# Amano-Ginji/distributed-tensorflow-example

Measured on AMD Instinct MI355X. Metric: samples/sec (whole node) MNIST MLP sync-SGD at 1/2/4/8 MI355X; step-time p50, higher is better.
Workload: dtype fp32; 1 GPU; model=mlp-784-100-10 (example.py), global_batch=100, per_gpu_batch=100, parallelism=dp1, optimizer=sgd lr=0.0005, grad_allreduce=none, engine=persistent-fp32, exchange_mode=persistent, launch=single process, steps_per_launch=550, hipgraph_steps=0, input_prefetch=in-kernel copier workgroups, activation=sigmoid

## Files before the change

### csrc/kernels/mlp_persist_f32.hip

```cpp
#include "common.h"
#include "mlp_api.h"

#include <atomic>

#include <cstdlib>

namespace dtfk {
namespace mlpf {

typedef __attribute__((ext_vector_type(4))) uint32_t u32x4;
typedef __attribute__((address_space(1))) unsigned gu32;

constexpr int DIN = 784, HID = 100, NCLS = 10;
constexpr int NJ = 7;
constexpr int NQ = 4;
constexpr int NTW = 2;
constexpr int NBT = 7;
constexpr int BROWS = 16 * NBT;
constexpr int XTS = 128;
constexpr int NCOMP = NJ * NQ;
constexpr int THREADS = 512;
constexpr int NCOP = 16;
constexpr int NCOPR = 14;
constexpr int RES_LR_BYTE = 124;
// ... 324 lines not shown
}

__device__ void copier(const Args& a, int cid, uint8_t* smem) {
  const int tid = threadIdx.x;
  const int B = a.B;
  if (tid == 0) { PRO(NCOMP + cid, 0); }
  for (int st = cid; st < a.next_steps; st += NCOP) {
    const uint8_t* src = a.host_next + (long long)st * a.rec_h;
    uint8_t* dst = a.stage_next + (long long)st * REC;
    constexpr int C16 = DIN / 16;
    for (int k = tid; k < BROWS * C16; k += THREADS) {
      const int row = k / C16, c = k % C16;
      uint4 v = make_uint4(0u, 0u, 0u, 0u);
      if (row < B) v = reinterpret_cast<const uint4*>(src)[row * C16 + c];
      *reinterpret_cast<uint4*>(smem + row * CROW + 16 * c) = v;
    }
    if (tid < 128) dst[XROW_BYTES + tid] = tid < B ? src[(long long)B * DIN + tid] : (uint8_t)0;
    __syncthreads();
    for (int k = tid; k < BROWS * C16; k += THREADS) {
      const int row = k / C16, c = k % C16;
      reinterpret_cast<uint4*>(dst)[row * C16 + c] = *reinterpret_cast<const uint4*>(smem + row * CROW + 16 * c);
    }
    __syncthreads();
  }
  if (tid == 0) { PRO(NCOMP + cid, 1); }
}

__device__ void copier_res(const Args& a, int cid, uint8_t* smem) {
  if (cid >= NCOPR) return;
  const int tid = threadIdx.x;
  constexpr int RR = 8;
  int* dec = reinterpret_cast<int*>(smem + RR * CROW);
  const int B = a.B;
  const int hb = (int)(2 * a.rec_h);
  const auto hrs = __builtin_amdgcn_make_buffer_rsrc(const_cast<uint8_t*>(a.host_recs), 0, hb, 0x00020000);
  for (int st = 0;; ++st) {
    const long long k = a.run0 + st;
    if (tid == 0) {
      int d = 1;
      const long long t0 = (long long)__builtin_amdgcn_s_memrealtime();
      const long long lim = cid == 0 ? a.idle : a.idle + a.timeout;
      for (;;) {
        const long long v = __hip_atomic_load(a.door, __ATOMIC_RELAXED, __HIP_MEMORY_SCOPE_SYSTEM);
        if (v < 0) { d = 0; break; }
        if (v > k) break;
        if (cid != 0 && __hip_atomic_load(a.dctr + 16, __ATOMIC_RELAXED, __HIP_MEMORY_SCOPE_AGENT) != 0u) { d = 0; break; }
        if ((long long)__builtin_amdgcn_s_memrealtime() - t0 > lim) { d = 0; break; }
        __builtin_amdgcn_s_sleep(1);
      }
      if (cid == 0 && !d) __hip_atomic_store(a.dctr + 16, 1u, __ATOMIC_RELAXED, __HIP_MEMORY_SCOPE_AGENT);
      if (cid == 0 && d) { RTS(k, 0); }
      *dec = d;
    }
    __syncthreads();
    if (*dec == 0) break;
    const int slot = (int)(k & 1);
    const int hbase = slot * (int)a.rec_h;
    const int r0 = RR * cid;
    uint8_t* dst = const_cast<uint8_t*>(a.stage) + (long long)(st & 1) * REC;
    constexpr int C16 = DIN / 16;
    constexpr int NLD = (RR * C16 + THREADS - 1) / THREADS;
    u32x4 hv[NLD];
    uint32_t lv = 0;
    if (cid == 0 && tid < 32) {
      if (4 * tid == RES_LR_BYTE)
        lv = __float_as_uint(__hip_atomic_load(a.host_lr + slot, __ATOMIC_RELAXED, __HIP_MEMORY_SCOPE_SYSTEM));
      else
        lv = __builtin_amdgcn_raw_buffer_load_b32(hrs, 4 * tid < B ? hbase + B * DIN + 4 * tid : OOB_OFF, 0, SYS);
    }
#pragma unroll
    for (int i = 0; i < NLD; ++i) {
      const int t = tid + i * THREADS;
      const int rr = t / C16, cc = t % C16;
      const int row = r0 + rr;
      hv[i] = __builtin_amdgcn_raw_buffer_load_b128(hrs, (t < RR * C16 && row < B) ? hbase + row * DIN + 16 * cc : OOB_OFF,
                                                    0, SYS);
    }
#pragma unroll
    for (int i = 0; i < NLD; ++i) {
      const int t = tid + i * THREADS;
      if (t < RR * C16) *reinterpret_cast<u32x4*>(smem + (t / C16) * CROW + 16 * (t % C16)) = hv[i];
    }
    __syncthreads();
    for (int t = tid; t < RR * C16; t += THREADS) {
      const int rr = t / C16, cc = t % C16;
      const u32x4 v = *reinterpret_cast<const u32x4*>(smem + rr * CROW + 16 * cc);
      __builtin_amdgcn_raw_buffer_store_b128(v, region_rsrc(dst, (int)REC), (r0 + rr) * DIN + 16 * cc, 0, 16);
    }
    if (cid == 0 && tid < 32) {
      uint32_t v = lv;
      if (4 * tid != RES_LR_BYTE) {
        const int nv = B - 4 * tid;
        if (nv < 4) v = nv <= 0 ? 0u : (v & ((1u << (8 * nv)) - 1u));
      }
      __builtin_amdgcn_raw_buffer_store_b32(v, region_rsrc(dst, (int)REC), (int)XROW_BYTES + 4 * tid, 0, 16);
    }
    asm volatile("s_waitcnt vmcnt(0)" ::: "memory");
    __syncthreads();
    if (tid == 0) {
      __hip_atomic_fetch_add(a.dctr, 1u, __ATOMIC_RELAXED, __HIP_MEMORY_SCOPE_AGENT);
      if (cid == 0) { RTS(k, 1); }
    }
  }
  if (cid == 0 && tid == 0)
    __hip_atomic_store(a.host_state, a.launch_id, __ATOMIC_RELAXED, __HIP_MEMORY_SCOPE_SYSTEM);
}

template <int ACT, int NW, bool SPLIT, bool RES, bool INS = false>
__device__ void compute(const Args& a, const int j, const int q, uint8_t* smem) {
  const int dbg = INS ? a.dbg : 0;
  constexpr bool MULTI = NW > 1;
  const int tid = threadIdx.x, lane = tid & 63, w = __builtin_amdgcn_readfirstlane(tid >> 6);
  const int r = lane & 15, g = lane >> 4;
  const int c = j * NQ + q;
  const int B = a.B;
  f32x4* zbuf = reinterpret_cast<f32x4*>(smem + L_ZBUF);
  float* a2T = reinterpret_cast<float*>(smem + L_A2T);
  float* dz2T = reinterpret_cast<float*>(smem + L_DZ2T);
  float* dz3T = reinterpret_cast<float*>(smem + L_DZ3T);
  float* w2s = reinterpret_cast<float*>(smem + L_W2);
  float* b1s = reinterpret_cast<float*>(smem + L_B1);
  float* b2s = reinterpret_cast<float*>(smem + L_B2);
  float* rdb2 = reinterpret_cast<float*>(smem + L_RDB2);
  int* abort_flag = reinterpret_cast<int*>(smem + L_FLAG);
  int* census = abort_flag + 1;
  uint16_t* dzp = reinterpret_cast<uint16_t*>(smem + L_DZP);
  if (tid == 0) { PROC(c, 0); }

  const int hid = 16 * j + r;
  const bool hv = hid < HID;
  const int nt = ntile(q);
  const bool tv0 = w < nt, tv1 = w + 8 < nt;
  const int ft0 = tile0(q) + w, ft1 = tile0(q) + (tv1 ? w + 8 : 0);
  auto tvk = [=](int k) { return k ? tv1 : tv0; };
  auto ftk = [=](int k) { return k ? ft1 : ft0; };
  float Wt[NTW][4];
  f32x4 wld[NTW];
  if constexpr (RES) {
#pragma unroll
    for (int k = 0; k < NTW; ++k)
#pragma unroll
      for (int e = 0; e < 4; ++e)
        Wt[k][e] = (tvk(k) && hv) ? a.params[(16 * ftk(k) + 4 * g + e) * HID + hid] : 0.f;
  } else if constexpr (MULTI) {
    const int u0 = 16 * j + 4 * (r & 3);
#pragma unroll
    for (int k = 0; k < NTW; ++k)
      wld[k] = (tvk(k) && u0 < HID)
                   ? *reinterpret_cast<const f32x4*>(a.params + (16 * ftk(k) + 4 * g + (r >> 2)) * HID + u0)
                   : f32x4{0.f, 0.f, 0.f, 0.f};
  } else {
    const int u0 = 16 * j + 4 * (r & 3);
    const auto rw1 = __builtin_amdgcn_make_buffer_rsrc(a.params, 0, DIN * HID * 4, 0x00020000);
#pragma unroll
    for (int k = 0; k < NTW; ++k)
      wld[k] = __builtin_bit_cast(
          f32x4, __builtin_amdgcn_raw_buffer_load_b128(
                     rw1, (tvk(k) && u0 < HID) ? ((16 * ftk(k) + 4 * g + (r >> 2)) * HID + u0) * 4 : OOB_OFF, 0, 0));
  }
  float pv = 0.f;
  if constexpr (MULTI) {
    if (tid < 256) {
      const int n = tid >> 4, cl = tid & 15;
      const int hn = 16 * j + n;
      pv = (hn < HID && cl < NCLS) ? a.p_w2[hn * NCLS + cl] : 0.f;
    } else if (tid < 272) {
      const int hn = 16 * j + (tid - 256);
      pv = hn < HID ? a.p_b1[hn] : 0.f;
    } else if (tid < 288) {
      const int cl = tid - 272;
      pv = cl < NCLS ? a.p_b2[cl] : 0.f;
    }
  } else {
    const int n = tid >> 4, cl = tid & 15, hn = 16 * j + n, hb = 16 * j + (tid - 256), c2 = tid - 272;
    const auto rw2 = __builtin_amdgcn_make_buffer_rsrc(a.p_w2, 0, HID * NCLS * 4, 0x00020000);
    const auto rb1 = __builtin_amdgcn_make_buffer_rsrc(a.p_b1, 0, HID * 4, 0x00020000);
    const auto rb2 = __builtin_amdgcn_make_buffer_rsrc(a.p_b2, 0, NCLS * 4, 0x00020000);
    const uint32_t v0 =
        __builtin_amdgcn_raw_buffer_load_b32(rw2, (tid < 256 && hn < HID && cl < NCLS) ? (hn * NCLS + cl) * 4 : OOB_OFF, 0, 0);
    const uint32_t v1 =
        __builtin_amdgcn_raw_buffer_load_b32(rb1, (tid >= 256 && tid < 272 && hb < HID) ? hb * 4 : OOB_OFF, 0, 0);
    const uint32_t v2 =
        __builtin_amdgcn_raw_buffer_load_b32(rb2, (tid >= 272 && tid < 288 && c2 < NCLS) ? c2 * 4 : OOB_OFF, 0, 0);
    pv = __uint_as_float(v0 | v1 | v2);
  }
  unsigned long long seq0 = *a.seq;
  long long gstep0 = *a.gstep;
  float lr = *a.lr;
  const unsigned xcc = __builtin_amdgcn_s_getreg((15 << 11) | (0 << 6) | 20) & 15u;
  unsigned long long* hdr = reinterpret_cast<unsigned long long*>(a.xbuf + HDR_OFF);
  const unsigned tag0 = a.census_tag;
  if (tid == 0)
    __hip_atomic_store(hdr + c, ((unsigned long long)tag0 << 32) | xcc, __ATOMIC_RELAXED, __HIP_MEMORY_SCOPE_AGENT);
  for (int k = tid; k < 3 * 16 * LS; k += THREADS) a2T[k] = 0.f;
  if constexpr (SPLIT)
    for (int k = tid; k < 3 * 16 * PS; k += THREADS) dzp[k] = (uint16_t)0;
  for (int k = tid; k < (XTS - BROWS) * XF_ROW / 16; k += THREADS)
    *reinterpret_cast<u32x4*>(smem + L_XF + BROWS * XF_ROW + 16 * k) = u32x4{0u, 0u, 0u, 0u};
  const bool failed_in = __hip_atomic_load(a.err, __ATOMIC_RELAXED, __HIP_MEMORY_SCOPE_AGENT) != 0;

  constexpr int XTN = SPLIT ? 8 : NBT;
  uint32_t xf[NTW][NBT], xt[NTW][XTN];
  int lab = 0;
  constexpr bool PREP = SPLIT && !RES && NW == 1;
  constexpr bool MET_FAST = PREP;
  bf16x8 XF[NBT], XA[NTW][4];
  int lab_n = 0;
  auto pin8 = [](bf16x8& v) {
    u32x4 t = __builtin_bit_cast(u32x4, v);
    asm volatile("" : "+v"(t));
    v = __builtin_bit_cast(bf16x8, t);
  };
  auto tlk = [=](int k) { return k ? (tv1 ? w + 8 : 0) : w; };
  auto stage_x = [&](int st, int n0, int dn) {
    const uint8_t* rec = a.stage + (long long)st * REC;
    const uint8_t* xr = rec + 16 * tile0(q);
#pragma unroll 1
    for (int n = n0; n < (XF_CHUNKS + 63) / 64; n += dn) {
      const int k = 64 * n + lane;
      if (k < XF_CHUNKS) glds16(xr + (k / 13) * DIN + 16 * (k % 13), smem + L_XF + 1024 * n);
    }
    if (n0 == 0 && lane < 8) glds16(rec + XROW_BYTES + 16 * lane, smem + L_LAB);
  };
  auto read_xf = [&](int& lb) {
#pragma unroll
    for (int k = 0; k < NTW; ++k)
#pragma unroll
      for (int b = 0; b < NBT; ++b)
        xf[k][b] = *reinterpret_cast<const uint32_t*>(smem + L_XF + (16 * b + r) * XF_ROW + 16 * tlk(k) + 4 * g);
    lb = smem[L_LAB + 16 * (w < NBT ? w : NBT - 1) + r];
  };
  auto read_xt = [&]() {
    typedef int v2i __attribute__((ext_vector_type(2)));
    typedef __attribute__((address_space(3))) v2i lds_v2i;
    const int row = SPLIT ? 8 * g + (r >> 1) : 16 * (r >> 3) + 4 * g + ((r >> 1) & 3);
#pragma unroll
    for (int k = 0; k < NTW; ++k) {
      const uint8_t* blk = smem + L_XF + row * XF_ROW + 16 * tlk(k) + 8 * (r & 1);
#pragma unroll
      for (int cc = 0; cc < 4; ++cc) {
        const v2i v = __builtin_amdgcn_ds_read_tr8_b64_v2i32((lds_v2i*)(blk + 32 * cc * XF_ROW));
        xt[k][2 * cc] = (uint32_t)v.x;
        if (2 * cc + 1 < XTN) xt[k][2 * cc + 1] = (uint32_t)v.y;
      }
    }
  };
  auto prep_fwd = [&](int& lb) {
    read_xf(lb);
#pragma unroll
    for (int b = 0; b < NBT; ++b) XF[b] = px8(xf[0][b], xf[1][b]);
#pragma unroll
    for (int b = 0; b < NBT; ++b) pin8(XF[b]);
    read_xt();
  };
  auto prep_xa = [&]() {
    if constexpr (SPLIT) {
#pragma unroll
      for (int k = 0; k < NTW; ++k)
#pragma unroll
        for (int i = 0; i < 8; ++i) asm volatile("" : "+v"(xt[k][i]));
#pragma unroll
      for (int ch = 0; ch < 4; ++ch) {
        XA[0][ch] = px8(xt[0][2 * ch], xt[0][2 * ch + 1]);
        XA[1][ch] = tv1 ? px8(xt[1][2 * ch], xt[1][2 * ch + 1]) : px8(0x01010101u, 0x01010101u);
      }
#pragma unroll
      for (int k = 0; k < NTW; ++k)
#pragma unroll
        for (int ch = 0; ch < 4; ++ch) pin8(XA[k][ch]);
    }
  };
  if (tid == 0) { PROC(c, 4); }
  if constexpr (!RES) stage_x(0, w, 8);
  if (w == 0) {
    const long long t0 = (long long)__builtin_amdgcn_s_memrealtime();
    unsigned long long v = 0;
    bool seen = lane >= NCOMP, bad = false;
    for (;;) {
      if (!seen) {
        v = __hip_atomic_load(hdr + lane, __ATOMIC_RELAXED, __HIP_MEMORY_SCOPE_AGENT);
        seen = (unsigned)(v >> 32) == tag0;
      }
      if (__all(seen)) break;
      if ((long long)__builtin_amdgcn_s_memrealtime() - t0 > a.timeout) {
        if (lane == 0) atomicOr(a.err, 1);
        bad = true;
        break;
      }
      __builtin_amdgcn_s_sleep(1);
    }
    const bool off = lane < NCOMP && (unsigned)v != xcc;
    const bool e1 = !__any(off && lane / NQ == j);
    const bool e2 = !__any(off && lane % NQ == q);
    if (lane == 0) *census = bad ? -1 : ((e1 ? 1 : 0) | (e2 ? 2 : 0));
  }
  if (tid < 256) {
    w2s[tid] = pv;
  } else if (tid < 272) {
    b1s[tid - 256] = pv;
  } else if (tid < 288) {
    b2s[tid - 272] = pv;
  } else if (tid == 288) {
    *abort_flag = 0;
  } else if (tid >= 296 && tid < 304) {
    reinterpret_cast<int*>(smem + L_HFLAG)[tid - 296] = 0;
  }
  asm volatile("s_waitcnt vmcnt(0)" ::: "memory");
  if constexpr (!MULTI) {
    asm volatile("" : "+v"(seq0), "+v"(gstep0), "+v"(lr));
    seq0 = ((unsigned long long)__builtin_amdgcn_readfirstlane((unsigned)(seq0 >> 32)) << 32) |
           __builtin_amdgcn_readfirstlane((unsigned)seq0);
    gstep0 = (long long)(((unsigned long long)__builtin_amdgcn_readfirstlane((unsigned)((unsigned long long)gstep0 >> 32))
                          << 32) |
                         __builtin_amdgcn_readfirstlane((unsigned)gstep0));
  }
  double gvar0 = 0.0;
  if constexpr (RES) {
    if (a.gvar_kind == 1) gvar0 = *static_cast<const float*>(a.gvar);
    else if (a.gvar_kind == 2) gvar0 = (double)*static_cast<const long long*>(a.gvar);
    else if (a.gvar_kind == 3) gvar0 = *static_cast<const int*>(a.gvar);
    else if (a.gvar_kind == 4) gvar0 = *static_cast<const double*>(a.gvar);
    else gvar0 = (double)gstep0;
  }
#pragma unroll
  for (int k = 0; k < NTW && !RES; ++k) {
    const int m = r & 3, b = r >> 2;
#pragma unroll
    for (int t = 0; t < 4; ++t) {
      const int cs = (b + t) & 3;
      const float v = cs == 0 ? wld[k][0] : (cs == 1 ? wld[k][1] : (cs == 2 ? wld[k][2] : wld[k][3]));
      const int e = (m - t) & 3;
      const float got = __shfl(v, 16 * g + 4 * e + b);
#pragma unroll
      for (int q = 0; q < 4; ++q)
        if (q == e) Wt[k][q] = got;
    }
  }
  __syncthreads();
  float lrB = lr / (float)(B * (MULTI ? a.W : 1));
  float lrX = lrB * (1.f / 255.f);
  if (failed_in || *census < 0) return;
  const bool l2_e1 = (*census & 1) != 0;
  const bool l2_e2 = (*census & 2) != 0;
  if (tid == 0) { PROC(c, 1); }
  if constexpr (PREP) {
    prep_fwd(lab);
  } else if constexpr (!RES) {
    read_xf(lab);
    read_xt();
  }
  if (tid == 0) { PROC(c, 2); }

  auto res_stage = [&](int st) -> bool {
    int* rflag = abort_flag + 2;
    if (tid == 0) {
      const unsigned need = (unsigned)NCOPR * (unsigned)(st + 1);
      const long long t0 = (long long)__builtin_amdgcn_s_memrealtime();
      int v = 1;
      for (;;) {
        if (__hip_atomic_load(a.dctr, __ATOMIC_RELAXED, __HIP_MEMORY_SCOPE_AGENT) >= need) break;
        if (__hip_atomic_load(a.dctr + 16, __ATOMIC_RELAXED, __HIP_MEMORY_SCOPE_AGENT) != 0u) { v = 0; break; }
        if ((long long)__builtin_amdgcn_s_memrealtime() - t0 > a.idle + a.timeout) {
          atomicOr(a.err, 4);
          v = 0;
          break;
        }
        __builtin_amdgcn_s_sleep(1);
      }
      *rflag = v;
    }
    __syncthreads();
    if (*rflag == 0) return false;
    if (c == 0 && tid == 0) { RTSC(a.run0 + st, 2); }
    const auto rs = region_rsrc(a.stage + (long long)(st & 1) * REC, (int)REC);
    const int xr0 = 16 * tile0(q);
#pragma unroll 4
    for (int k = tid; k < XF_CHUNKS; k += THREADS) {
      const u32x4 v = __builtin_amdgcn_raw_buffer_load_b128(rs, (k / 13) * DIN + 16 * (k % 13) + xr0, 0, 16);
      *reinterpret_cast<u32x4*>(smem + L_XF + 16 * k) = v;
    }
    if (tid < 8) {
      const u32x4 v = __builtin_amdgcn_raw_buffer_load_b128(rs, (int)XROW_BYTES + 16 * tid, 0, 16);
      *reinterpret_cast<u32x4*>(smem + L_LAB + 16 * tid) = v;
    }
    __syncthreads();
    read_xf(lab);
    read_xt();
    if (c == 0 && tid == 0) { RTSC(a.run0 + st, 3); }
    const float lr_run = *reinterpret_cast<const float*>(smem + L_LAB + RES_LR_BYTE);
    lrB = lr_run / (float)B;
    lrX = lrB * (1.f / 255.f);
    return true;
  };
  int st_done = 0;
  auto write_params = [&](bool wt) {
    auto put = [wt](float* p, float v) {
      if (wt) __hip_atomic_store(p, v, __ATOMIC_RELAXED, __HIP_MEMORY_SCOPE_AGENT);
      else *p = v;
    };
    if (hv) {
#pragma unroll
      for (int k = 0; k < NTW; ++k)
        if (tvk(k)) {
#pragma unroll
          for (int e = 0; e < 4; ++e) put(a.params + (16 * ftk(k) + 4 * g + e) * HID + hid, Wt[k][e]);
        }
    }
    if (q == 0) {
      if (tid < 256) {
        const int n = tid >> 4, cl = tid & 15;
        const int hn = 16 * j + n;
        if (hn < HID && cl < NCLS) put(a.p_w2 + hn * NCLS + cl, w2s[tid]);
      } else if (tid < 272) {
        const int hn = 16 * j + (tid - 256);
        if (hn < HID) put(a.p_b1 + hn, b1s[tid - 256]);
      }
    }
    if (c == 0 && tid >= 272 && tid < 272 + NCLS) put(a.p_b2 + (tid - 272), b2s[tid - 272]);
  };

  unsigned mslot0 = 0u;
  if constexpr (MET_FAST) {
    if (c == 0) mslot0 = (unsigned)(gstep0 % a.ring);
  }

  const PeerRs<NW> prs = peer_rsrcs<NW>(a.peer_base, MULTI ? a.W : 1);
  bool aborted = false;
  for (int st = 0; st < a.nsteps; ++st) {
    if constexpr (RES) {
      if (!res_stage(st)) break;
    }
    int jq[2] = {j, q};
    asm volatile("" : "+s"(jq[0]), "+s"(jq[1]));
    const unsigned long long sq = seq0 + (unsigned long long)st + 1ull;
    const unsigned tag = (unsigned)sq;
    const int par = (int)(sq & 1ull);
    if (c == 0 && tid == 0 && a.step_ts != nullptr)
      a.step_ts[(gstep0 + st) % a.ts_ring] = (long long)__builtin_amdgcn_s_memrealtime();
    if (w == 0) { PH(0); }
    if (w == 7) { PH7(14); }

    {
      f32x4 acc[NBT];
#pragma unroll
      for (int b = 0; b < NBT; ++b) acc[b] = f32x4{0.f, 0.f, 0.f, 0.f};
      if constexpr (SPLIT) {
        float wv[8];
#pragma unroll
        for (int i = 0; i < 8; ++i) wv[i] = Wt[i >> 2][i & 3];
        bf16x8 Ah, Am, Al;
        split8(wv, Ah, Am, Al);
        bf16x8 X[NBT];
#pragma unroll
        for (int b = 0; b < NBT; ++b) {
          if constexpr (PREP) X[b] = XF[b];
          else X[b] = px8(xf[0][b], xf[1][b]);
        }
#pragma unroll
        for (int b = 0; b < NBT; ++b) acc[b] = mfma16x16x32(Al, X[b], acc[b]);
#pragma unroll
        for (int b = 0; b < NBT; ++b) acc[b] = mfma16x16x32(Am, X[b], acc[b]);
#pragma unroll
        for (int b = 0; b < NBT; ++b) acc[b] = mfma16x16x32(Ah, X[b], acc[b]);
      } else {
#pragma unroll
        for (int k = 0; k < NTW; ++k) {
          if (tvk(k)) {
#pragma unroll
            for (int e = 0; e < 4; ++e)
#pragma unroll
              for (int b = 0; b < NBT; ++b) acc[b] = mfma4(Wt[k][e], ub(xf[k][b], e), acc[b]);
          }
        }
      }
#pragma unroll
      for (int b = 0; b < NBT; ++b) zbuf[(w * NBT + b) * 64 + lane] = acc[b];
    }
    if (w == 0) { PH(1); }
    PHB(w);
    lds_barrier();
    if (w == 0) { PH(2); }
    const bool more = !RES && st + 1 < a.nsteps;
    int* hflag = reinterpret_cast<int*>(smem + L_HFLAG);
    auto heads_done = [&]() -> unsigned {
      const bool ok = lane < NBT && __hip_atomic_load(hflag + (lane < NBT ? lane : 0), __ATOMIC_RELAXED,
                                                      __HIP_MEMORY_SCOPE_WORKGROUP) >= st + 1;
      return (unsigned)__ballot(ok) & ((1u << NBT) - 1u);
    };
    if (w == 7 && more && !(dbg & 1)) {
      stage_x(st + 1, 0, 1);
      asm volatile("s_waitcnt vmcnt(0)" ::: "memory");
      __builtin_amdgcn_fence(__ATOMIC_RELEASE, "workgroup", "local");
      if (lane == 0) __hip_atomic_store(hflag + 7, st + 1, __ATOMIC_RELAXED, __HIP_MEMORY_SCOPE_WORKGROUP);
      if ((dbg & 8) == 0) { PH7(15); }
    } else if (w == 7 && more && lane == 0) {
      __hip_atomic_store(hflag + 7, st + 1, __ATOMIC_RELAXED, __HIP_MEMORY_SCOPE_WORKGROUP);
    }
    bool prepped = false;
    if constexpr (PREP) {
      if (w == 7) {
        prep_xa();
        if (more && !(dbg & 4)) {
          __builtin_amdgcn_fence(__ATOMIC_ACQUIRE, "workgroup", "local");
          prep_fwd(lab_n);
          prepped = true;
        }
      }
    }

    if (w < NBT) {
      const int bw = 16 * w + r;
      const bool bv = bw < B;
      f32x4 zs = zbuf[w * 64 + lane];
#pragma unroll
      for (int v = 1; v < 8; ++v) zs += zbuf[(v * NBT + w) * 64 + lane];
      const auto r1 = region_rsrc(a.xbuf + E1_OFF + (long long)(par * NJ + j) * NQ * NBT * GSLOT, NQ * NBT * GSLOT);
      put_gran(r1, (q * NBT + w) * GSLOT + 32 * lane, zs, tag, l2_e1);
      if (w == 0) { PH(3); }
      if constexpr (PREP) prep_xa();
      float w2p[4], w2d[4], b1v[4], b2v[4];
#pragma unroll
      for (int e = 0; e < 4; ++e) {
        w2p[e] = w2s[(4 * g + e) * 16 + r];
        w2d[e] = w2s[r * 16 + 4 * g + e];
        b1v[e] = b1s[4 * g + e];
        b2v[e] = b2s[4 * g + e];
      }
      f32x4 part[NQ];
      bool ok = gather_gran<NQ>(r1, [&](int k) { return (k * NBT + w) * GSLOT; }, jq[1], true, tag, zs, part, lane, a);
      f32x4 z = part[0];
#pragma unroll
      for (int qq = 1; qq < NQ; ++qq) z += part[qq];
      if (w == 0) { PH(4); }
      if (w == 0) { PH(5); }
      float a2[4];
#pragma unroll
      for (int i = 0; i < 4; ++i) {
        const int hl = 4 * g + i;
        const float zt = z[i] * (1.f / 255.f) + b1v[i];
        const float av = ACT == 0 ? __builtin_amdgcn_rcpf(1.f + __expf(-zt)) : fmaxf(zt, 0.f);
        a2[i] = (16 * j + hl < HID) ? av : 0.f;
      }
      f32x4 pl = {0.f, 0.f, 0.f, 0.f};
#pragma unroll
      for (int e = 0; e < 4; ++e) pl = mfma4(w2p[e], a2[e], pl);
      const auto r2 = region_rsrc(a.xbuf + E2_OFF + (long long)((par * NQ + q) * NBT + w) * NJ * GSLOT, NJ * GSLOT);
      if (g < 3) put_gran(r2, j * GSLOT + 32 * lane, pl, tag, l2_e2);
      if (w == 0) { PH(6); }
#pragma unroll
      for (int i = 0; i < 4; ++i) a2T[(4 * g + i) * LS + bw] = a2[i];
      f32x4 lp[NJ];
      ok = gather_gran<NJ>(r2, [&](int k) { return k * GSLOT; }, jq[0], g < 3, tag, pl, lp, lane, a) && ok;
      if (w == 0) { PH(7); }
      if (!ok && lane == 0) *abort_flag = 1;
      float lg[4], ex[4];
      float m = -3.0e38f;
#pragma unroll
      for (int i = 0; i < 4; ++i) {
        float v = b2v[i];
#pragma unroll
        for (int jj = 0; jj < NJ; ++jj) v += lp[jj][i];
        lg[i] = v;
        if (4 * g + i < NCLS) m = fmaxf(m, v);
      }
      if (w == 0) { PH(8); }
      m = fmaxf(m, xor16(m));
      m = fmaxf(m, xor32(m));
      const int y = lab < NCLS ? lab : 0;
      float ssum = 0.f, zy = 0.f, am = 1e9f;
#pragma unroll
      for (int i = 0; i < 4; ++i) {
        const int cl = 4 * g + i;
        ex[i] = cl < NCLS ? __expf(lg[i] - m) : 0.f;
        ssum += ex[i];
        zy += (cl == y) ? lg[i] : 0.f;
        if (cl < NCLS && lg[i] == m) am = fminf(am, (float)cl);
      }
      ssum += xor16(ssum); ssum += xor32(ssum);
      zy += xor16(zy); zy += xor32(zy);
      am = fminf(am, xor16(am)); am = fminf(am, xor32(am));
      const float inv = __builtin_amdgcn_rcpf(ssum);
      if (w == 0) { PHX(13); }
      float dz3[4], py = 0.f;
#pragma unroll
      for (int i = 0; i < 4; ++i) {
        const int cl = 4 * g + i;
        const float p = ex[i] * inv;
        py += (cl == y) ? p : 0.f;
        dz3[i] = (bv && cl < NCLS) ? p - (cl == y ? 1.f : 0.f) : 0.f;
      }
      py += xor16(py); py += xor32(py);
      const float loss = a.naive ? -__logf(py) : (m + __logf(ssum) - zy);
      f32x4 da = {0.f, 0.f, 0.f, 0.f};
#pragma unroll
      for (int e = 0; e < 4; ++e) da = mfma4(w2d[e], dz3[e], da);
      if (w == 0) { PHX(14); }
#pragma unroll
      for (int i = 0; i < 4; ++i) {
        const float d = ACT == 0 ? da[i] * a2[i] * (1.f - a2[i]) : (a2[i] > 0.f ? da[i] : 0.f);
        if constexpr (SPLIT) {
          uint32_t ph, pm, pl;
          split3(d, ph, pm, pl);
          const int o = (4 * g + i) * PS + bw;
          dzp[o] = (uint16_t)(ph >> 16);
          dzp[16 * PS + o] = (uint16_t)(pm >> 16);
          dzp[32 * PS + o] = (uint16_t)(pl >> 16);
        } else {
          dz2T[(4 * g + i) * LS + bw] = d;
        }
        dz3T[(4 * g + i) * LS + bw] = dz3[i];
      }
      if (w == 0) { PHX(15); }
      if (g == 0) {
        float* rl = reinterpret_cast<float*>(smem + L_RLOSS);
        rl[bw] = bv ? loss : 0.f;
        rl[128 + bw] = (bv && (int)am == y) ? 1.f : 0.f;
      }
      asm volatile("s_waitcnt lgkmcnt(0)" ::: "memory");
      {
        const f32x4 av = *reinterpret_cast<const f32x4*>(a2T + r * LS + 16 * w + 4 * g);
        const f32x4 dv = *reinterpret_cast<const f32x4*>(dz3T + r * LS + 16 * w + 4 * g);
        const float one = r == 0 ? 1.f : 0.f;
        f32x4 dp = {0.f, 0.f, 0.f, 0.f}, p2 = dp;
#pragma unroll
        for (int e = 0; e < 4; ++e) {
          dp = mfma4(av[e], dv[e], dp);
          p2 = mfma4(one, dv[e], p2);
        }
        reinterpret_cast<f32x4*>(smem + L_DW2P)[w * 64 + lane] = dp;
        if (g == 0) rdb2[w * 16 + r] = p2[0];
      }
      __builtin_amdgcn_fence(__ATOMIC_RELEASE, "workgroup", "local");
      if (lane == 0)
        __hip_atomic_store(reinterpret_cast<int*>(smem + L_HFLAG) + w, st + 1, __ATOMIC_RELAXED,
                           __HIP_MEMORY_SCOPE_WORKGROUP);
      if (w == 0) { PH(9); }
      PHB(8 + w);
    }
    f32x4 G[NTW];
    f32x4 G1[NTW];
#pragma unroll
    for (int k = 0; k < NTW; ++k) G[k] = G1[k] = f32x4{0.f, 0.f, 0.f, 0.f};
    constexpr int NCH = SPLIT ? 4 : NBT;
    auto need_of = [](int ch) -> unsigned {
      return SPLIT ? ((1u << (2 * ch)) | (2 * ch + 1 < NBT ? 1u << (2 * ch + 1) : 0u)) : (1u << ch);
    };
    auto chunk = [&](int ch) {
      if constexpr (SPLIT) {
        const uint16_t* bp = dzp + r * PS + 32 * ch + 8 * g;
        const bf16x8 Bh = *reinterpret_cast<const bf16x8*>(bp);
        const bf16x8 Bm = *reinterpret_cast<const bf16x8*>(bp + 16 * PS);
        const bf16x8 Bl = *reinterpret_cast<const bf16x8*>(bp + 32 * PS);
        bf16x8 X0, X1;
        if constexpr (PREP) X0 = XA[0][ch];
        else X0 = px8(xt[0][2 * ch], xt[0][2 * ch + 1]);
        if (tv1 || w == 7) {
          if constexpr (PREP) X1 = XA[1][ch];
          else X1 = tv1 ? px8(xt[1][2 * ch], xt[1][2 * ch + 1]) : px8(0x01010101u, 0x01010101u);
          G[0] = mfma16x16x32(X0, Bl, G[0]);
          G[1] = mfma16x16x32(X1, Bl, G[1]);
          G[0] = mfma16x16x32(X0, Bm, G[0]);
          G[1] = mfma16x16x32(X1, Bm, G[1]);
          G[0] = mfma16x16x32(X0, Bh, G[0]);
          G[1] = mfma16x16x32(X1, Bh, G[1]);
        } else {
          G[0] = mfma16x16x32(X0, Bl, G[0]);
          G[0] = mfma16x16x32(X0, Bm, G[0]);
          G[0] = mfma16x16x32(X0, Bh, G[0]);
        }
      } else {
        const f32x4 bz = *reinterpret_cast<const f32x4*>(dz2T + r * LS + 16 * ch + 4 * g);
#pragma unroll
        for (int k = 0; k < NTW; ++k) {
          if (tvk(k)) {
            G[k] = mfma4(ub(xt[k][ch], 0), bz[0], G[k]);
            G1[k] = mfma4(ub(xt[k][ch], 1), bz[1], G1[k]);
            G[k] = mfma4(ub(xt[k][ch], 2), bz[2], G[k]);
            G1[k] = mfma4(ub(xt[k][ch], 3), bz[3], G1[k]);
          }
        }
        if (w == 7) {
          G[1] = mfma4(1.f, bz[0], G[1]);
          G1[1] = mfma4(1.f, bz[1], G1[1]);
          G[1] = mfma4(1.f, bz[2], G[1]);
          G1[1] = mfma4(1.f, bz[3], G1[1]);
        }
      }
    };
    {
      int cc = 0;
      for (;;) {
        const unsigned hm = heads_done();
        bool did = false;
#pragma unroll
        for (int ch = 0; ch < NCH; ++ch) {
          if (ch == cc && (hm & need_of(ch)) == need_of(ch)) {
            if (!did) __builtin_amdgcn_fence(__ATOMIC_ACQUIRE, "workgroup", "local");
            if (cc == 0 && w == 0) { PH(10); }
            chunk(ch);
            ++cc;
            did = true;
          }
        }
        if (cc == NCH) break;
        if (!did) __builtin_amdgcn_s_sleep(0);
      }
    }
    if constexpr (!SPLIT) {
#pragma unroll
      for (int k = 0; k < NTW; ++k) G[k] = G[k] + G1[k];
    }
    f32x4 D = {0.f, 0.f, 0.f, 0.f};
    float gb = 0.f;
    if (w == 7) {
      if constexpr (INS) {
        if ((dbg & 8) != 0) { PH7(15); }
      }
      const float* gsrc = rdb2 + (lane >= 16 && lane < 16 + NCLS ? lane - 16 : 0);
      const f32x4* dw2p = reinterpret_cast<const f32x4*>(smem + L_DW2P);
#pragma unroll
      for (int v = 0; v < NBT; ++v) {
        D += dw2p[v * 64 + lane];
        gb += gsrc[v * 16];
      }
      if (lane < 16) gb = G[1][0];
      if (lane >= 16 + NCLS) gb = 0.f;
      PH7(13);
      if (c == 0) {
        const float* rl = reinterpret_cast<const float*>(smem + L_RLOSS);
        const bool hi = lane + 64 < BROWS;
        auto wsum = [&](float v) {
          if constexpr (MET_FAST) {
            v += xor32(v);
            v += xor16(v);
            return row16_sum(v);
          } else {
            return wave_sum(v);
          }
        };
        const float ls = wsum(rl[lane] + (hi ? rl[lane + 64] : 0.f));
        const float cr = wsum(rl[128 + lane] + (hi ? rl[128 + lane + 64] : 0.f));
        if (lane == 63) {
          const int sl = MET_FAST ? (int)((mslot0 + (unsigned)st) % (unsigned)a.ring) : (int)((gstep0 + st) % a.ring);
          if constexpr (RES) {
            reinterpret_cast<float*>(abort_flag)[4] = ls / (float)B;
            reinterpret_cast<float*>(abort_flag)[5] = cr / (float)B;
            __hip_atomic_store(a.metrics + 2 * sl, ls / (float)B, __ATOMIC_RELAXED, __HIP_MEMORY_SCOPE_AGENT);
            __hip_atomic_store(a.metrics + 2 * sl + 1, cr / (float)B, __ATOMIC_RELAXED, __HIP_MEMORY_SCOPE_AGENT);
          } else {
            a.metrics[2 * sl] = ls / (float)B;
            a.metrics[2 * sl + 1] = cr / (float)B;
          }
        }
      }
      if constexpr (!MULTI) {
#pragma unroll
        for (int i = 0; i < 4; ++i)
          if (16 * j + 4 * g + i < HID && r < NCLS) w2s[(4 * g + i) * 16 + r] -= lrB * D[i];
        if (lane < 16) {
          if (16 * j + lane < HID) b1s[lane] -= lrB * gb;
        } else if (lane < 16 + NCLS) {
          b2s[lane - 16] -= lrB * gb;
        }
      }
      PHB(15);
    }
    if (*abort_flag) { aborted = true; break; }
    if (more && !prepped) {
      while (__hip_atomic_load(hflag + 7, __ATOMIC_RELAXED, __HIP_MEMORY_SCOPE_WORKGROUP) < st + 1)
        __builtin_amdgcn_s_sleep(1);
      __builtin_amdgcn_fence(__ATOMIC_ACQUIRE, "workgroup", "local");
      if constexpr (PREP) {
        prep_fwd(lab_n);
      } else {
        read_xf(lab);
        read_xt();
      }
    }
    if constexpr (PREP) lab = lab_n;
    if (w == 0) { PH(11); }
    if constexpr (MULTI) {
      const bool pk = a.gbf16 != 0;
      const size_t soff = IPC_FLAGS + (size_t)(par * NCOMP + c) * IPC_SLOT;
      char* own = static_cast<char*>(a.peer_base[a.rank]) + soff;
      const int eb = (w * 64 + lane) * 16;
      const int ef0 = ((w * NTW + 0) * 64 + lane) * 16;
      const int ef1 = ((w * NTW + 1) * 64 + lane) * 16;
      const bool dlane = r < NCLS && 16 * j + 4 * g < HID;
      const bool blane = lane < 16 ? 16 * j + lane < HID : lane < 16 + NCLS;
      if (hv) {
        if (pk) {
          const uint32_t p0 = pack2bf(G[0][0], G[0][1]), p1 = pack2bf(G[0][2], G[0][3]);
          const uint32_t p2 = pack2bf(G[1][0], G[1][1]), p3 = pack2bf(G[1][2], G[1][3]);
          if (tv1) *reinterpret_cast<uint4*>(own + eb) = make_uint4(p0, p1, p2, p3);
          else if (tv0) *reinterpret_cast<uint2*>(own + eb) = make_uint2(p0, p1);
        } else {
          if (tv0) *reinterpret_cast<f32x4*>(own + ef0) = G[0];
          if (tv1) *reinterpret_cast<f32x4*>(own + ef1) = G[1];
        }
      }
      if (pk) {
        G[0] = round_bf16x4(G[0]);
        G[1] = round_bf16x4(G[1]);
      }
      if (w == 7) {
        if (dlane) *reinterpret_cast<f32x4*>(own + IPC_SMALL + lane * 16) = D;
        if (blane) *reinterpret_cast<float*>(own + IPC_SMALL + 1024 + lane * 4) = gb;
      }
      asm volatile("s_waitcnt vmcnt(0)" ::: "memory");
      lds_barrier();
      char* flags = static_cast<char*>(a.peer_base[a.rank]);
      auto wait_peers = [&](int fo) {
        if (w == 0) {
          const long long t0 = (long long)__builtin_amdgcn_s_memrealtime();
          for (;;) {
            bool ok = true;
            if (lane < a.W && lane != a.rank) {
              const unsigned v = __hip_atomic_load(
                  reinterpret_cast<const unsigned*>(static_cast<const char*>(a.peer_base[lane]) + 64 * c + fo),
                  __ATOMIC_RELAXED, __HIP_MEMORY_SCOPE_SYSTEM);
              ok = (int)(v - tag) >= 0;
            }
            if (__all(ok)) break;
            if ((long long)__builtin_amdgcn_s_memrealtime() - t0 > a.timeout ||
                __hip_atomic_load(a.err, __ATOMIC_RELAXED, __HIP_MEMORY_SCOPE_AGENT) != 0) {
              if (lane == 0) {
                atomicOr(a.err, 2);
                *abort_flag = 1;
              }
              break;
            }
            __builtin_amdgcn_s_sleep(1);
          }
        }
        lds_barrier();
        asm volatile("" ::: "memory");
      };
      if (tid == 0 && !(a.rank == a.fault_rank && gstep0 + st >= a.fault_step))
        __hip_atomic_store(reinterpret_cast<unsigned*>(flags + 64 * c), tag, __ATOMIC_RELAXED,
                           __HIP_MEMORY_SCOPE_SYSTEM);
      wait_peers(0);
      if (*abort_flag) { aborted = true; break; }
      auto sum_ranks = [&](size_t so) {
        constexpr int GF = NW < 4 ? NW : 4;
        if (pk) {
          if (tv1) sum_entries<NW, NW, true, true>(prs, a.W, a.rank, (int)so, hv, eb, eb, G[0], G[1]);
          else sum_entries<NW, NW, true, false>(prs, a.W, a.rank, (int)so, hv, eb, eb, G[0], G[1]);
        } else {
          if (tv1) sum_entries<NW, GF, false, true>(prs, a.W, a.rank, (int)so, hv, ef0, ef1, G[0], G[1]);
          else sum_entries<NW, GF, false, false>(prs, a.W, a.rank, (int)so, hv, ef0, ef1, G[0], G[1]);
        }
        if (w == 7) sum_small<NW>(prs, a.W, a.rank, (int)so + IPC_SMALL, dlane, blane, lane, D, gb);
      };
      if (a.xmode == 0) {
        sum_ranks(soff);
      } else {
        const int own_chunk = w % a.W;
        const size_t roff = IPC_RED + (size_t)(par * NCOMP + c) * IPC_SLOT;
        char* ored = static_cast<char*>(a.peer_base[a.rank]) + roff;
        if (own_chunk == a.rank) {
          sum_ranks(soff);
          if (hv) {
            if (pk) {
              const uint32_t p0 = pack2bf(G[0][0], G[0][1]), p1 = pack2bf(G[0][2], G[0][3]);
              const uint32_t p2 = pack2bf(G[1][0], G[1][1]), p3 = pack2bf(G[1][2], G[1][3]);
              if (tv1) *reinterpret_cast<uint4*>(ored + eb) = make_uint4(p0, p1, p2, p3);
              else if (tv0) *reinterpret_cast<uint2*>(ored + eb) = make_uint2(p0, p1);
              G[0] = round_bf16x4(G[0]);
              G[1] = round_bf16x4(G[1]);
            } else {
              if (tv0) *reinterpret_cast<f32x4*>(ored + ef0) = G[0];
              if (tv1) *reinterpret_cast<f32x4*>(ored + ef1) = G[1];
            }
          }
          if (w == 7) {
            if (dlane) *reinterpret_cast<f32x4*>(ored + IPC_SMALL + lane * 16) = D;
            if (blane) *reinterpret_cast<float*>(ored + IPC_SMALL + 1024 + lane * 4) = gb;
          }
        }
        asm volatile("s_waitcnt vmcnt(0)" ::: "memory");
        lds_barrier();
        if (tid == 0)
          __hip_atomic_store(reinterpret_cast<unsigned*>(flags + 64 * c + 8), tag, __ATOMIC_RELAXED,
                             __HIP_MEMORY_SCOPE_SYSTEM);
        wait_peers(8);
        if (*abort_flag) { aborted = true; break; }
        if (own_chunk != a.rank) {
          __amdgpu_buffer_rsrc_t rs = prs.r[0];
#pragma unroll
          for (int rr = 1; rr < NW; ++rr)
            if (rr == own_chunk) rs = prs.r[rr];
          const int ro = (int)roff;
          if (pk) {
            if (tv1) {
              const u32x4 v = __builtin_amdgcn_raw_buffer_load_b128(rs, hv ? ro + eb : OOB_OFF, 0, SYS);
              G[0] = unbf4(v[0], v[1]);
              G[1] = unbf4(v[2], v[3]);
            } else {
              const u32x2 v = __builtin_amdgcn_raw_buffer_load_b64(rs, hv ? ro + eb : OOB_OFF, 0, SYS);
              G[0] = unbf4(v[0], v[1]);
            }
          } else {
            G[0] = __builtin_bit_cast(f32x4, __builtin_amdgcn_raw_buffer_load_b128(rs, hv ? ro + ef0 : OOB_OFF, 0, SYS));
            if (tv1)
              G[1] = __builtin_bit_cast(f32x4, __builtin_amdgcn_raw_buffer_load_b128(rs, hv ? ro + ef1 : OOB_OFF, 0, SYS));
          }
          if (w == 7) {
            D = __builtin_bit_cast(
                f32x4, __builtin_amdgcn_raw_buffer_load_b128(rs, dlane ? ro + IPC_SMALL + lane * 16 : OOB_OFF, 0, SYS));
            gb = __uint_as_float(
                __builtin_amdgcn_raw_buffer_load_b32(rs, blane ? ro + IPC_SMALL + 1024 + lane * 4 : OOB_OFF, 0, SYS));
          }
        }
      }
    }
    if (hv) {
#pragma unroll
      for (int k = 0; k < NTW; ++k)
#pragma unroll
        for (int i = 0; i < 4; ++i) Wt[k][i] -= (k == 0 || tv1) ? lrX * G[k][i] : 0.f;
    }
    if (w == 0) { PH(12); }
    if (MULTI && w == 7) {
#pragma unroll
      for (int i = 0; i < 4; ++i)
        if (16 * j + 4 * g + i < HID && r < NCLS) w2s[(4 * g + i) * 16 + r] -= lrB * D[i];
      if (lane < 16) {
        if (16 * j + lane < HID) b1s[lane] -= lrB * gb;
      } else if (lane < 16 + NCLS) {
        b2s[lane - 16] -= lrB * gb;
      }
    }
    st_done = st + 1;
    if constexpr (RES) {
      __syncthreads();
      if (c == 0 && tid == 0) { RTSC(a.run0 + st, 4); }
      write_params(true);
      const double gsv = gvar0 + (double)(st + 1);
      if (c == 0 && tid == 0) {
        if (a.gvar_kind == 1) __hip_atomic_store(static_cast<float*>(a.gvar), (float)gsv, __ATOMIC_RELAXED, __HIP_MEMORY_SCOPE_AGENT);
        else if (a.gvar_kind == 2) __hip_atomic_store(static_cast<long long*>(a.gvar), (long long)gsv, __ATOMIC_RELAXED, __HIP_MEMORY_SCOPE_AGENT);
        else if (a.gvar_kind == 3) __hip_atomic_store(static_cast<int*>(a.gvar), (int)gsv, __ATOMIC_RELAXED, __HIP_MEMORY_SCOPE_AGENT);
        else if (a.gvar_kind == 4) __hip_atomic_store(static_cast<double*>(a.gvar), gsv, __ATOMIC_RELAXED, __HIP_MEMORY_SCOPE_AGENT);
      }
      asm volatile("s_waitcnt vmcnt(0)" ::: "memory");
      __syncthreads();
      if (tid == 0) {
        if (c == 0) { RTSC(a.run0 + st, 5); }
        __hip_atomic_fetch_add(a.dctr + 32, 1u, __ATOMIC_RELAXED, __HIP_MEMORY_SCOPE_AGENT);
        if (c == 0) {
          const unsigned need = (unsigned)NCOMP * (unsigned)(st + 1);
          const long long t0 = (long long)__builtin_amdgcn_s_memrealtime();
          while (__hip_atomic_load(a.dctr + 32, __ATOMIC_RELAXED, __HIP_MEMORY_SCOPE_AGENT) < need) {
            if ((long long)__builtin_amdgcn_s_memrealtime() - t0 > a.timeout) {
              atomicOr(a.err, 8);
              break;
            }
          }
          RTSC(a.run0 + st, 6);
          const float* mf = reinterpret_cast<const float*>(abort_flag);
          __hip_atomic_store(a.host_out, mf[4], __ATOMIC_RELAXED, __HIP_MEMORY_SCOPE_SYSTEM);
          __hip_atomic_store(a.host_out + 1, mf[5], __ATOMIC_RELAXED, __HIP_MEMORY_SCOPE_SYSTEM);
          __hip_atomic_store(a.host_out + 2, (float)gsv, __ATOMIC_RELAXED, __HIP_MEMORY_SCOPE_SYSTEM);
          asm volatile("s_waitcnt vmcnt(0)" ::: "memory");
          __hip_atomic_store(a.host_done, a.run0 + st + 1, __ATOMIC_RELAXED, __HIP_MEMORY_SCOPE_SYSTEM);
          RTSC(a.run0 + st, 7);
        }
      }
    }
  }
  if (aborted) return;
  __syncthreads();
  if (tid == 0) { PROC(c, 3); }

  write_params(false);
  if (c == 0 && tid == 300) {
    *a.gstep = gstep0 + st_done;
    *a.seq = seq0 + (unsigned long long)st_done;
    if (a.step_ts != nullptr)
      a.step_ts[(gstep0 + st_done) % a.ts_ring] = (long long)__builtin_amdgcn_s_memrealtime();
  }
  if (tid == 0) { PROC(c, 5); }
}

template <int ACT, int NW, bool SPLIT, bool RES = false, bool INS = false>
__global__ __launch_bounds__(THREADS, 1) void mlp_persist_f32(Args a) {
  extern __shared__ __attribute__((aligned(16))) uint8_t smem[];
  const int b = blockIdx.x;
  int c = -1, cid = -1;
  if (a.spread) {
    if (b < NCOMP) c = b; else cid = b - NCOMP;
  } else {
    if ((b & 7) == 0) c = b >> 3; else cid = b - (b >> 3) - 1;
  }
  if (c >= 0) {
    if (a.nsteps > 0) compute<ACT, NW, SPLIT, RES, INS>(a, c / NQ, c % NQ, smem);
    return;
  }
  if constexpr (RES) copier_res(a, cid, smem);
  else if (cid < NCOP) copier(a, cid, smem);
}

static int g_fault_rank = -1;
static long long g_fault_step = -1;

static unsigned next_census_tag() {
  static std::atomic<unsigned> ctr{0};
  unsigned t = ctr.fetch_add(1u, std::memory_order_relaxed) + 1u;
  return t == 0u ? ctr.fetch_add(1u, std::memory_order_relaxed) + 1u : t;
}

static int persist_dbg() {
  static const int dbg = [] {
    const char* db = getenv("DTF_PERSIST_DBG");
    return db ? atoi(db) : 0;
  }();
  return dbg;
}

static Args make_args(const Launch& p) {
// ... 115 lines not shown
```

### distributed_tensorflow_example_amd/utils/graphs.py

```python
from __future__ import annotations

from collections import OrderedDict
from typing import Callable, List, Sequence

import torch


class _Captured:
    __slots__ = ("graph", "static_in", "out")

    def __init__(self, graph, static_in, out):
        self.graph, self.static_in, self.out = graph, static_in, out


class GraphedStep:

    def __init__(self, step_fn: Callable, state: Callable[[], Sequence[torch.Tensor]], warmup: int = 2,
                 strict: bool = False, max_graphs: int = 8):
        self.step_fn = step_fn
        self.state = state
        self.warmup = warmup
        self.strict = strict
        self.max_graphs = 1 if strict else max(1, int(max_graphs))
        self._graphs: "OrderedDict[tuple, _Captured]" = OrderedDict()
        self.captures = 0
        self.replays = 0

    @staticmethod
    def _sig(inputs):
        return tuple((tuple(t.shape), t.dtype, t.device) for t in inputs)

    @property
    def key(self):
        return next(reversed(self._graphs)) if self._graphs else None

    @property
    def graph(self):
        return self._graphs[self.key].graph if self._graphs else None

    @property
    def out(self):
        return self._graphs[self.key].out if self._graphs else None

    def _capture(self, inputs):
        sig = self._sig(inputs)
        self._graphs.pop(sig, None)
        static_in = [t.detach().clone() for t in inputs]
        saved = [t.detach().clone() for t in self.state()]
        cur = torch.cuda.current_stream()
        side = torch.cuda.Stream()
        side.wait_stream(cur)
        with torch.cuda.stream(side):
            for _ in range(self.warmup):
                self.step_fn(*static_in)
        cur.wait_stream(side)
        from .. import ops
        g = torch.cuda.CUDAGraph()
        ops.bump_capture_epoch()
        with torch.cuda.graph(g):
            out = self.step_fn(*static_in)
        ops.bump_capture_epoch()
        with torch.no_grad():
            for t, s in zip(self.state(), saved):
                t.copy_(s)
        del saved
        self._graphs[sig] = _Captured(g, static_in, out)
        while len(self._graphs) > self.max_graphs:
            self._graphs.popitem(last=False)
        self.captures += 1

    def capture(self, *inputs):
        if self.strict:
            self._graphs.clear()
        self._capture(inputs)

    def matches(self, *inputs) -> bool:
        return self._sig(inputs) in self._graphs

    def __call__(self, *inputs):
        sig = self._sig(inputs)
        c = self._graphs.get(sig)
        if c is None:
            if self.strict:
                raise RuntimeError("captured multi-rank step called with other input shapes "
                                   f"({sig} vs {self.key}): pad inputs to the static capacity; a "
                                   "re-capture must be collective (capture() on every rank)")
            self._capture(inputs)
            c = self._graphs[sig]
        else:
            self._graphs.move_to_end(sig)
        with torch.no_grad():
            from .. import ops
            ops.multi_copy_(c.static_in, inputs)
        c.graph.replay()
        self.replays += 1
        return c.out
```

Baseline: 15.09 million samples/s.

## Publish head-done flag before loss/accuracy math and add second flag set for dW2 partials

The output-layer head now signals completion to the waiting stage right after writing the backward deltas, before computing loss, argmax accuracy and writing the dW2/db2 partials. Those are guarded by a second set of workgroup flags (offset 8), which the consumer polls before reading the partial sums. Loss and accuracy work is moved off the critical path so the next phase can start sooner. The cost is extra flag traffic and a spin-wait, and the wider flag initialisation region must not collide with other LDS data. The graph capture code also disables Python GC during capture, which is a robustness change.

```diff
diff --git a/csrc/kernels/mlp_persist_f32.hip b/csrc/kernels/mlp_persist_f32.hip
--- a/csrc/kernels/mlp_persist_f32.hip
+++ b/csrc/kernels/mlp_persist_f32.hip
@@ -650,7 +650,7 @@
     b2s[tid - 272] = pv;
   } else if (tid == 288) {
     *abort_flag = 0;
-  } else if (tid >= 296 && tid < 304) {
+  } else if (tid >= 296 && tid < 312) {
     reinterpret_cast<int*>(smem + L_HFLAG)[tid - 296] = 0;
   }
   asm volatile("s_waitcnt vmcnt(0)" ::: "memory");
@@ -830,11 +830,13 @@
     if (w == 0) { PH(2); }
     const bool more = !RES && st + 1 < a.nsteps;
     int* hflag = reinterpret_cast<int*>(smem + L_HFLAG);
-    auto heads_done = [&]() -> unsigned {
-      const bool ok = lane < NBT && __hip_atomic_load(hflag + (lane < NBT ? lane : 0), __ATOMIC_RELAXED,
+    auto flags_up = [&](int f0) -> unsigned {
+      const bool ok = lane < NBT && __hip_atomic_load(hflag + f0 + (lane < NBT ? lane : 0), __ATOMIC_RELAXED,
                                                       __HIP_MEMORY_SCOPE_WORKGROUP) >= st + 1;
       return (unsigned)__ballot(ok) & ((1u << NBT) - 1u);
     };
+    const int chunk_flag = (dbg & 16) != 0 ? 8 : 0;
+    auto heads_done = [&]() -> unsigned { return flags_up(chunk_flag); };
     if (w == 7 && more && !(dbg & 1)) {
       stage_x(st + 1, 0, 1);
       asm volatile("s_waitcnt vmcnt(0)" ::: "memory");
@@ -915,30 +917,23 @@
       m = fmaxf(m, xor16(m));
       m = fmaxf(m, xor32(m));
       const int y = lab < NCLS ? lab : 0;
-      float ssum = 0.f, zy = 0.f, am = 1e9f;
+      float ssum = 0.f;
+#pragma unroll
+      for (int i = 0; i < 4; ++i) {
+        ex[i] = 4 * g + i < NCLS ? __expf(lg[i] - m) : 0.f;
+        ssum += ex[i];
+      }
+      ssum += xor16(ssum); ssum += xor32(ssum);
+      const float inv = __builtin_amdgcn_rcpf(ssum);
+      if (w == 0) { PHX(13); }
+      float pr[4], dz3[4];
 #pragma unroll
       for (int i = 0; i < 4; ++i) {
         const int cl = 4 * g + i;
-        ex[i] = cl < NCLS ? __expf(lg[i] - m) : 0.f;
-        ssum += ex[i];
-        zy += (cl == y) ? lg[i] : 0.f;
-        if (cl < NCLS && lg[i] == m) am = fminf(am, (float)cl);
-      }
-      ssum += xor16(ssum); ssum += xor32(ssum);
-      zy += xor16(zy); zy += xor32(zy);
-      am = fminf(am, xor16(am)); am = fminf(am, xor32(am));
-      const float inv = __builtin_amdgcn_rcpf(ssum);
-      if (w == 0) { PHX(13); }
-      float dz3[4], py = 0.f;
-#pragma unroll
-      for (int i = 0; i < 4; ++i) {
-        const int cl = 4 * g + i;
-        const float p = ex[i] * inv;
-        py += (cl == y) ? p : 0.f;
-        dz3[i] = (bv && cl < NCLS) ? p - (cl == y ? 1.f : 0.f) : 0.f;
-      }
-      py += xor16(py); py += xor32(py);
-      const float loss = a.naive ? -__logf(py) : (m + __logf(ssum) - zy);
+        pr[i] = ex[i] * inv;
+        asm("" : "+v"(pr[i]));
+        dz3[i] = (bv && cl < NCLS) ? pr[i] - (cl == y ? 1.f : 0.f) : 0.f;
+      }
       f32x4 da = {0.f, 0.f, 0.f, 0.f};
 #pragma unroll
       for (int e = 0; e < 4; ++e) da = mfma4(w2d[e], dz3[e], da);
@@ -959,10 +954,37 @@
         dz3T[(4 * g + i) * LS + bw] = dz3[i];
       }
       if (w == 0) { PHX(15); }
-      if (g == 0) {
-        float* rl = reinterpret_cast<float*>(smem + L_RLOSS);
-        rl[bw] = bv ? loss : 0.f;
-        rl[128 + bw] = (bv && (int)am == y) ? 1.f : 0.f;
+      __builtin_amdgcn_fence(__ATOMIC_RELEASE, "workgroup", "local");
+      if (lane == 0) __hip_atomic_store(hflag + w, st + 1, __ATOMIC_RELAXED, __HIP_MEMORY_SCOPE_WORKGROUP);
+      if (w == 0) { PH(9); }
+      PHB(8 + w);
+      if (c == 0) {
+        int ym = y;
+        asm volatile("" : "+v"(ym));
+        float zy = 0.f, am = 1e9f;
+#pragma unroll
+        for (int i = 0; i < 4; ++i) {
+          const int cl = 4 * g + i;
+          zy += (cl == ym) ? lg[i] : 0.f;
+          if (cl < NCLS && lg[i] == m) am = fminf(am, (float)cl);
+        }
+        zy += xor16(zy); zy += xor32(zy);
+        am = fminf(am, xor16(am)); am = fminf(am, xor32(am));
+        float loss;
+        if (a.naive) {
+          float py = 0.f;
+#pragma unroll
+          for (int i = 0; i < 4; ++i) py += (4 * g + i == ym) ? pr[i] : 0.f;
+          py += xor16(py); py += xor32(py);
+          loss = -__logf(py);
+        } else {
+          loss = m + __logf(ssum) - zy;
+        }
+        if (g == 0) {
+          float* rl = reinterpret_cast<float*>(smem + L_RLOSS);
+          rl[bw] = bv ? loss : 0.f;
+          rl[128 + bw] = (bv && (int)am == ym) ? 1.f : 0.f;
+        }
       }
       asm volatile("s_waitcnt lgkmcnt(0)" ::: "memory");
       {
@@ -979,11 +1001,7 @@
         if (g == 0) rdb2[w * 16 + r] = p2[0];
       }
       __builtin_amdgcn_fence(__ATOMIC_RELEASE, "workgroup", "local");
-      if (lane == 0)
-        __hip_atomic_store(reinterpret_cast<int*>(smem + L_HFLAG) + w, st + 1, __ATOMIC_RELAXED,
-                           __HIP_MEMORY_SCOPE_WORKGROUP);
-      if (w == 0) { PH(9); }
-      PHB(8 + w);
+      if (lane == 0) __hip_atomic_store(hflag + 8 + w, st + 1, __ATOMIC_RELAXED, __HIP_MEMORY_SCOPE_WORKGROUP);
     }
     f32x4 G[NTW];
     f32x4 G1[NTW];
@@ -1064,6 +1082,8 @@
       if constexpr (INS) {
         if ((dbg & 8) != 0) { PH7(15); }
       }
+      while (flags_up(8) != (1u << NBT) - 1u) __builtin_amdgcn_s_sleep(0);
+      __builtin_amdgcn_fence(__ATOMIC_ACQUIRE, "workgroup", "local");
       const float* gsrc = rdb2 + (lane >= 16 && lane < 16 + NCLS ? lane - 16 : 0);
       const f32x4* dw2p = reinterpret_cast<const f32x4*>(smem + L_DW2P);
 #pragma unroll
diff --git a/distributed_tensorflow_example_amd/utils/graphs.py b/distributed_tensorflow_example_amd/utils/graphs.py
--- a/distributed_tensorflow_example_amd/utils/graphs.py
+++ b/distributed_tensorflow_example_amd/utils/graphs.py
@@ -1,5 +1,6 @@
 from __future__ import annotations
 
+import gc
 from collections import OrderedDict
 from typing import Callable, List, Sequence
 
@@ -57,8 +58,15 @@
         from .. import ops
         g = torch.cuda.CUDAGraph()
         ops.bump_capture_epoch()
-        with torch.cuda.graph(g):
-            out = self.step_fn(*static_in)
+        gc_on = gc.isenabled()
+        gc.collect()
+        gc.disable()
+        try:
+            with torch.cuda.graph(g):
+                out = self.step_fn(*static_in)
+        finally:
+            if gc_on:
+                gc.enable()
         ops.bump_capture_epoch()
         with torch.no_grad():
             for t, s in zip(self.state(), saved):
```

Result: faster. 15.68 million samples/s, median of 6 (+3.9%).
